# tuannv-github/srsRAN_Project

Hardware: AMD Instinct MI355X
Metric: PDSCH+PUSCH codeblocks/s @ 100 MHz 273-PRB 4x4 MIMO (PDSCH 4 layers, PUSCH 4 layers x 4 rx) (higher is better)
Workload: dtype int8+fp32; 1 GPU; BASELINE metric (PDSCH+PUSCH codeblocks/s @ 100 MHz 273-PRB 4x4 MIMO): full PDSCH+PUSCH slot pipeline, 100 MHz numerology-1 273 PRB, 256QAM R=948/1024; parallelism=single GPU

## Files before the change

### srsran_project_amd/csrc/ldpc_api.cpp

```cpp
#include "srsran_amd/ldpc.h"

#include <hip/hip_runtime.h>

#include "api_common.h"
#include "ldpc_codec_internal.h"
#include "ldpc_common.h"
#include <cstdarg>
#include <cstdio>
#include <cstring>
#include <mutex>
#include <string>
#include <algorithm>
#include <vector>

namespace srs_amd {


hipError_t launch_ldpc_decode(const decode_args& args, const lifted_graph& g, int arith, int grid, hipStream_t stream);
size_t     ldpc_decode_lds_bytes(const lifted_graph& g);

namespace {

constexpr int      MAX_CRC_BITS_LEN = 22 * MAX_LIFTING_SIZE;
constexpr uint32_t DEFAULT_SLOTS    = 1u << 20;
// ... 180 lines not shown
{
  return srs_amd::ldpc_decode_batch_ex(d, cfg, crc_poly, d_llrs, llr_stride, d_llr_lens, llr_len, d_output,
                                       out_stride, d_nof_iters, d_soft_out, nof_cbs, stream, nullptr, 0);
}

}

int srs_amd::ldpc_decode_batch_ex(srs_amd_ldpc_decoder*              d,
                                  const srs_amd_ldpc_decoder_config* cfg,
                                  int                                crc_poly,
                                  const int8_t*                      d_llrs,
                                  uint32_t                           llr_stride,
                                  const uint32_t*                    d_llr_lens,
                                  uint32_t                           llr_len,
                                  uint8_t*                           d_output,
                                  uint32_t                           out_stride,
                                  int32_t*                           d_nof_iters,
                                  int8_t*                            d_soft_out,
                                  uint32_t                           nof_cbs,
                                  void*                              stream,
                                  const uint8_t*                     d_skip_flags,
                                  uint32_t                           skip_stride,
                                  const int32_t*                     d_fillers,
                                  const ldpc_cw_rows*                cw)
{
  if (d == nullptr) {
    return fail(SRS_AMD_EINVAL, "null decoder");
  }
  int rc = validate(cfg, crc_poly);
  if (rc != SRS_AMD_OK) {
    return rc;
  }
  const uint32_t Z       = cfg->lifting_size;
  const uint32_t K       = (cfg->base_graph == 1 ? 22 : 10) * Z;
  const uint32_t N_short = (cfg->base_graph == 1 ? 66 : 50) * Z;
  if (nof_cbs == 0) {
    return SRS_AMD_OK;
  }
  if ((d_llrs == nullptr && cw == nullptr) || d_output == nullptr || d_nof_iters == nullptr ||
      (cw != nullptr && (cw->llrs == nullptr || cw->offsets == nullptr || cw->lengths == nullptr))) {
    return fail(SRS_AMD_EINVAL, "null device buffer");
  }
  if (cw != nullptr && (d_llr_lens != nullptr || d_soft_out != nullptr || d_skip_flags != nullptr || cw->qm == 0 ||
                        !ldpc_hr_takes(static_cast<int>(cfg->base_graph), static_cast<int>(cfg->lifting_size), llr_len))) {
    return fail(SRS_AMD_EINVAL, "codeword-fed rows need the high-rate decoder's configuration");
  }
  if (out_stride < (K + 7) / 8) {
// ... 27 lines not shown
  a.edges = d->edges + ((cfg->base_graph - 1) * NOF_LIFTING_SIZES + lifting_size_position(static_cast<int>(Z))) *
                             static_cast<size_t>(MAX_EDGES);
  a.llr_stride      = llr_stride;
  a.aligned4        = ((reinterpret_cast<uintptr_t>(d_llrs) | llr_stride) & 3u) == 0 ? 1 : 0;
  a.llr_len         = llr_len;
  a.out_stride      = out_stride;
  a.nof_cbs         = nof_cbs;
  a.nof_filler_bits = static_cast<int32_t>(cfg->nof_filler_bits);
  a.max_iterations  = static_cast<int32_t>(cfg->max_iterations);
  a.force_decoding  = d->force_decoding;
  a.skip_flags      = d_skip_flags;
  a.skip_stride     = skip_stride;
  a.fillers         = d_fillers;
  if (cw != nullptr) {
    a.llrs        = cw->llrs;
    a.aligned4    = 1;
    a.cw_llrs     = cw->llrs;
    a.cw_offsets  = cw->offsets;
    a.cw_lengths  = cw->lengths;
    a.cw_qm       = cw->qm;
    a.cw_nof_info = cw->nof_info;
    a.cw_filler   = cw->filler;
  }
  const int grid    = static_cast<int>(nof_cbs < d->max_slots ? nof_cbs : d->max_slots);
  e = launch_ldpc_decode(a, g, d->arith, grid, static_cast<hipStream_t>(stream));
  if (e != hipSuccess) {
    return hip_fail(e, "ldpc_decode_kernel launch");
  }
  return SRS_AMD_OK;
}

void srs_amd::ldpc_mixed_row(void* row, uint32_t bg, uint32_t Z, int crc_poly)
{
  ldpc_row_desc r{};
  r.Z        = Z;
  r.edge_off = static_cast<uint32_t>(lifted_edges_offset(static_cast<int>(bg), static_cast<int>(Z)));
  r.crc_off  = crc_poly == SRS_AMD_NO_CRC ? NO_CRC_ROW : static_cast<uint32_t>(crc_poly) * MAX_CRC_BITS_LEN;
  r.zmagic   = ldpc_z_magic(Z);
  std::memcpy(row, &r, sizeof(r));
}

int srs_amd::ldpc_decode_mixed(srs_amd_ldpc_decoder* d,
                               uint32_t              bg,
                               uint32_t              max_z,
                               uint32_t              max_iterations,
                               const int8_t*         d_llrs,
// ... 114 lines not shown
```

### srsran_project_amd/csrc/ldpc_codec_internal.h

```cpp
#pragma once

#include "srsran_amd/ldpc.h"
#include "srsran_amd/ldpc_encoder.h"
#include "srsran_amd/ldpc_rate_matching.h"

namespace srs_amd {

int rate_dematch_batch_ex(srs_amd_ldpc_rate_dematcher*      dm,
                          const srs_amd_codeblock_metadata* cfg,
                          int                               new_data,
                          const int8_t*                     d_input,
                          const uint32_t*                   d_in_offsets,
                          const uint32_t*                   d_rm_lengths,
                          int8_t*                           d_soft,
                          uint32_t                          soft_stride,
                          uint32_t                          nof_cbs,
                          void*                             stream,
                          bool                              fresh,
                          uint32_t                          write_end = 0);

int ldpc_encode_batch_ex(srs_amd_ldpc_encoder*              enc,
                         const srs_amd_ldpc_encoder_config* cfg,
                         const uint8_t*                     d_messages,
                         uint32_t                           msg_stride,
// ... 6 lines not shown
struct ldpc_cw_rows {
  const int8_t*   llrs;
  const uint32_t* offsets;
  const uint32_t* lengths;
  uint32_t        qm, nof_info, filler;
};

int ldpc_decode_batch_ex(srs_amd_ldpc_decoder*              d,
                         const srs_amd_ldpc_decoder_config* cfg,
                         int                                crc_poly,
                         const int8_t*                      d_llrs,
                         uint32_t                           llr_stride,
                         const uint32_t*                    d_llr_lens,
                         uint32_t                           llr_len,
                         uint8_t*                           d_output,
                         uint32_t                           out_stride,
                         int32_t*                           d_nof_iters,
                         int8_t*                            d_soft_out,
                         uint32_t                           nof_cbs,
                         void*                              stream,
                         const uint8_t*                     d_skip_flags,
                         uint32_t                           skip_stride,
                         const int32_t*                     d_fillers = nullptr,
                         const ldpc_cw_rows*                cw        = nullptr);

int ldpc_decode_mixed(srs_amd_ldpc_decoder* d,
                      uint32_t              bg,
                      uint32_t              max_z,
                      uint32_t              max_iterations,
                      const int8_t*         d_llrs,
                      uint32_t              llr_stride,
                      const uint32_t*       d_llr_lens,
                      uint8_t*              d_output,
                      uint32_t              out_stride,
                      int32_t*              d_nof_iters,
                      uint32_t              nof_cbs,
                      void*                 stream,
                      const int32_t*        d_fillers,
                      const void*           d_rows);

void ldpc_mixed_row(void* row, uint32_t bg, uint32_t Z, int crc_poly);

int ldpc_encode_mixed(srs_amd_ldpc_encoder* enc,
                      uint32_t              bg,
                      uint32_t              max_z,
                      uint32_t              max_rows_eff,
                      const uint8_t*        d_messages,
// ... 38 lines not shown
```

### srsran_project_amd/csrc/ldpc_common.h

```cpp
#pragma once

#include <cstddef>
#include <cstdint>
#include <vector>

namespace srs_amd {

constexpr int LLR_MAX      = 120;
constexpr int LLR_INFINITY = 127;
constexpr int SOFT_CLAMP = 64;

constexpr int MAX_LIFTING_SIZE = 384;
constexpr int MAX_BG_M         = 46;
constexpr int MAX_BG_N_FULL    = 68;
constexpr int MAX_EDGES        = 316;
constexpr int BG1_MAX_DEGREE   = 19;
constexpr int BG2_MAX_DEGREE   = 10;

enum arith_flavour : int {
  ARITH_SIMD = 0,
  ARITH_GENERIC = 1,
};

struct lifted_graph {
// ... 14 lines not shown
  uint8_t*        out;
  int32_t*        nof_iters;
  int8_t*         soft_out;
  const uint32_t* crc_table;
  const uint32_t* edges;
  uint32_t        llr_stride;
  uint32_t        llr_len;
  uint32_t        out_stride;
  uint32_t        nof_cbs;
  int32_t         nof_filler_bits;
  int32_t         max_iterations;
  int32_t         force_decoding;
  int32_t         aligned4;
  const uint8_t*  skip_flags;
  uint32_t        skip_stride;
  const int32_t*  fillers;
  const struct ldpc_row_desc* rows;
  const int8_t*   cw_llrs;
  const uint32_t* cw_offsets;
  const uint32_t* cw_lengths;
  uint32_t        cw_qm;
  uint32_t        cw_nof_info;
  uint32_t        cw_filler;
};

struct ldpc_row_desc {
  uint32_t Z;
  uint32_t edge_off;
  uint32_t crc_off;
  uint32_t zmagic;
};

uint32_t ldpc_z_magic(uint32_t Z);

bool ldpc_hr_takes(int bg, int Z, uint32_t llr_len);

int ldpc_pk_waves(int bg, int Z);
constexpr uint32_t NO_CRC_ROW = 0xffffffffu;
constexpr int32_t LDPC_ITERS_SKIPPED = -2;

int lifting_size_position(int Z);
constexpr int NOF_LIFTING_SIZES = 51;

bool build_lifted_graph(lifted_graph& g, int bg, int Z);

std::vector<uint32_t> all_lifted_edges();

// ... 13 lines not shown
```

### srsran_project_amd/csrc/ldpc_decoder.hip

```cpp
#include "kernel_probe.h"
#include "srsran_amd/profiling.h"
#include <hip/hip_runtime.h>

#include "ldpc_common.h"
#include <cstdlib>
#include <type_traits>
#include <utility>

namespace srs_amd {

#define SRS_BG_TABLE_QUAL constexpr
namespace tables {
#include "bg_tables.inc"
}
#undef SRS_BG_TABLE_QUAL

using const_u32_ptr = const __attribute__((address_space(4))) uint32_t*;

constexpr int LDS_RED_OFFSET  = 16;
constexpr int LDS_SOFT_OFFSET = 80;
using lds_i8                  = __attribute__((address_space(3))) int8_t;
using lds_i32                 = __attribute__((address_space(3))) int32_t;
using lds_u32                 = __attribute__((address_space(3))) uint32_t;

// ... 594 lines not shown

__device__ __forceinline__ pk16 pk_splat(int v)
{
  return pk16{static_cast<short>(v), static_cast<short>(v)};
}
__device__ __forceinline__ pk16 pk_min(pk16 a, pk16 b)
{
  return __builtin_elementwise_min(a, b);
}
__device__ __forceinline__ pk16 pk_max(pk16 a, pk16 b)
{
  return __builtin_elementwise_max(a, b);
}
__device__ __forceinline__ pk16 pk_clamp(pk16 x, int lim)
{
  return pk_min(pk_max(x, pk_splat(-lim)), pk_splat(lim));
}

template <int MAXL>
__host__ __device__ constexpr int hr_lds_bytes()
{
  return LDS_SOFT_OFFSET + (22 + MAXL) * HR_Z;
}

template <int EI, int H, int KOFF = 0>
__device__ __forceinline__ uint32_t hr_addr(uint32_t t)
{
  constexpr uint32_t s    = (const_edge<1, HR_Z, EI>::shift + H) % HR_Z;
  constexpr uint32_t base = LDS_SOFT_OFFSET + const_edge<1, HR_Z, EI>::var * HR_Z;
  if constexpr (s <= HR_HALF) {
    return t + (base + KOFF + s);
  } else {
    return __builtin_elementwise_min(t + (KOFF + s), t + (KOFF + s - HR_Z)) + base;
  }
}

template <int N, typename F, int... I>
__device__ __forceinline__ void static_for_impl(F&& f, std::integer_sequence<int, I...>)
{
  (f(std::integral_constant<int, I>{}), ...);
}
template <int N, typename F>
__device__ __forceinline__ void static_for(F&& f)
{
  static_for_impl<N>(f, std::make_integer_sequence<int, N>{});
}
// ... 564 lines not shown
  uint32_t l;
  asm volatile("v_mbcnt_lo_u32_b32 %0, -1, 0\n\tv_mbcnt_hi_u32_b32 %0, -1, %0" : "=v"(l));
  return wave_base + l;
}

template <int ARITH, int MAXL, int NP>
__global__ void __launch_bounds__(HR_HALF / NP, (hr_waves_per_simd<NP, MAXL>())) ldpc_decode_hr_kernel(decode_args a)
{
  constexpr bool FULL   = MAXL == bg_traits<1>::M;
  constexpr bool CMP    = FULL || (HR_CMP && NP == 1);
  static_assert(!FULL || NP == 1, "full-length codeblocks: one row pair per lane");
  constexpr int Z       = HR_Z;
  constexpr int K       = 22 * Z;
  constexpr int NODES   = 22 + MAXL;
  constexpr int NE      = row_start<1>(MAXL) * NP;
  constexpr int MAX_LLR = (NODES - 2) * Z;
  constexpr int NT      = HR_HALF / NP;
  lds_i32*      red     = (lds_i32*)(uintptr_t)LDS_RED_OFFSET;
  lds_i8*       lds     = (lds_i8*)(uintptr_t)0;
  lds_i8*       soft    = lds + LDS_SOFT_OFFSET;
  lds_i32*      soft4   = reinterpret_cast<lds_i32*>(soft);

  const uint32_t wave_base = __builtin_amdgcn_readfirstlane(threadIdx.x) & ~63u;
  for (uint32_t cb = blockIdx.x; cb < a.nof_cbs; cb += gridDim.x) {
    uint32_t t = hr_thread(wave_base);
    if (a.skip_flags && *reinterpret_cast<const int32_t*>(a.skip_flags + static_cast<size_t>(cb) * a.skip_stride)) {
      if (t == 0) {
        a.nof_iters[cb] = LDPC_ITERS_SKIPPED;
      }
      continue;
    }
    asm volatile("" : "+v"(t));
    const int8_t* in     = a.llrs + static_cast<size_t>(cb) * a.llr_stride;
    const int     n_llrs = static_cast<int>(a.llr_len);
    uint8_t*      out    = a.out + static_cast<size_t>(cb) * a.out_stride;

    if constexpr (NT > 64) {
      if (t == 0) {
        red[0] = -1;
        red[1] = 0;
        red[2] = 0;
      }
      __syncthreads();
    }
    int input_size;
    if (a.cw_llrs != nullptr) {
// ... 264 lines not shown
        if (crc != 0) {
          __hip_atomic_fetch_xor(&acc[0], crc, __ATOMIC_RELAXED, __HIP_MEMORY_SCOPE_WORKGROUP);
        }
        if (zero != 0) {
          __hip_atomic_fetch_or(&acc[1], 1u, __ATOMIC_RELAXED, __HIP_MEMORY_SCOPE_WORKGROUP);
        }
        __syncthreads();
        const uint32_t c_all = __builtin_amdgcn_readfirstlane(acc[0]);
        const uint32_t z_all = __builtin_amdgcn_readfirstlane(acc[1]);
        if (tq == 0) {
          lds_u32* nxt = reinterpret_cast<lds_u32*>(&red[1 + 2 * ((it + 1) & 1)]);
          nxt[0]       = 0;
          nxt[1]       = 0;
        }
        if (z_all == 0 && c_all == 0) {
          result = it + 1;
          break;
        }
      }
    }

    const uint32_t te = hr_thread(wave_base);
    static_assert(K % 128 == 0, "whole 16-byte hard-decision tasks");
    for (int task = te; task < K / 128; task += NT) {
      uint32_t o[4];
#pragma unroll
      for (int c = 0; c < 4; ++c) {
        o[c] = 0;
#pragma unroll
        for (int h = 0; h < 8; ++h) {
          const uint32_t w = static_cast<uint32_t>(soft4[32 * task + 8 * c + h]);
          const uint32_t d    = ((w | 0x80808080u) - 0x01010101u) ^ (~w & 0x80808080u);
          const uint32_t nib  = (((d & 0x80808080u) >> 7) * 0x08040201u) >> 24;
          const int      byte = h >> 1;
          o[c] |= (nib & 0xfu) << (8 * byte + ((h & 1) ? 0 : 4));
        }
      }
      uint8_t* ob = out + 16 * task;
      if (((reinterpret_cast<uintptr_t>(ob)) & 15u) == 0) {
        *reinterpret_cast<uint4*>(ob) = uint4{o[0], o[1], o[2], o[3]};
      } else {
#pragma unroll
        for (int b = 0; b < 16; ++b) {
          ob[b] = static_cast<uint8_t>(o[b >> 2] >> (8 * (b & 3)));
        }
      }
    }
    if (a.soft_out) {
      int32_t* so = reinterpret_cast<int32_t*>(a.soft_out + static_cast<size_t>(cb) * (68 * Z));
      for (int i = te; i < 68 * Z / 4; i += NT) {
        so[i] = i < NODES * Z / 4 ? static_cast<int32_t>(soft_export4(static_cast<uint32_t>(soft4[i]))) : 0;
      }
    }
    if (te == 0) {
      a.nof_iters[cb] = result;
    }
    if constexpr (NT > 64) {
      __syncthreads();
    } else {
      asm volatile("" ::: "memory");
    }
  }
}


template <int BG>
constexpr int pk_words(int l)
{
  return bg_traits<BG>::deg(l) > 13 ? 3 : 2;
}
template <int BG>
constexpr int pk_off(int l)
{
  int s = 0;
  for (int i = 0; i < l; ++i) {
    s += pk_words<BG>(i);
  }
  return s;
}
static_assert(pk_off<1>(46) == FR_STATE_WORDS && pk_off<2>(42) == 84, "compressed message state");

// ... 454 lines not shown
  const size_t lds = lds_total_bytes<BG>(g.Z);
  if (g.Z == 384) {
    hipLaunchKernelGGL((ldpc_decode_kernel<BG, ARITH, 384>), dim3(grid), dim3(max_threads<384>()), lds, stream, args, g);
  } else {
    hipLaunchKernelGGL((ldpc_decode_kernel<BG, ARITH, 0>), dim3(grid), dim3(threads), lds, stream, args, g);
  }
}

bool ldpc_hr_takes(int bg, int Z, uint32_t llr_len)
{
  static const bool enabled = [] {
    const char* e = std::getenv("SRSRAN_AMD_LDPC_HR");
    return e == nullptr || e[0] != '0';
  }();
  return enabled && bg == 1 && Z == HR_Z && llr_len <= static_cast<uint32_t>((20 + HR_MAXL) * HR_Z) &&
         (llr_len & 3u) == 0;
}

hipError_t launch_ldpc_decode(const decode_args& args, const lifted_graph& g, int arith, int grid, hipStream_t stream)
{
  if (args.cw_llrs != nullptr && !(ldpc_decode_hr_eligible(args, g) && ldpc_hr_takes(g.bg, g.Z, args.llr_len))) {
    return hipErrorInvalidValue;
  }
  if (ldpc_decode_hr_eligible(args, g)) {
    constexpr size_t lds = hr_lds_bytes<HR_MAXL>();
    constexpr int    NT  = HR_HALF / HR_NP;
    if (arith == ARITH_GENERIC) {
      SRS_PROBED_LAUNCH(SRS_AMD_PROBE_LDPC_HR, (ldpc_decode_hr_kernel<ARITH_GENERIC, HR_MAXL, HR_NP>), dim3(grid),
                        dim3(NT), lds, stream, args);
    } else {
      SRS_PROBED_LAUNCH(SRS_AMD_PROBE_LDPC_HR, (ldpc_decode_hr_kernel<ARITH_SIMD, HR_MAXL, HR_NP>), dim3(grid),
                        dim3(NT), lds, stream, args);
    }
    return hipGetLastError();
  }
  if (ldpc_decode_full_eligible(args, g)) {
    constexpr int    MAXL = bg_traits<1>::M;
    constexpr size_t lds  = hr_lds_bytes<MAXL>();
    if (arith == ARITH_GENERIC) {
      SRS_PROBED_LAUNCH(SRS_AMD_PROBE_LDPC_FULL, (ldpc_decode_hr_kernel<ARITH_GENERIC, MAXL, 1>), dim3(grid),
                        dim3(HR_HALF), lds, stream, args);
    } else {
      SRS_PROBED_LAUNCH(SRS_AMD_PROBE_LDPC_FULL, (ldpc_decode_hr_kernel<ARITH_SIMD, MAXL, 1>), dim3(grid),
                        dim3(HR_HALF), lds, stream, args);
    }
    return hipGetLastError();
  }
  const int pkw = ldpc_pk_waves(g.bg, g.Z);
  if (pkw > 0 && !(g.bg == 1 && g.Z == HR_Z) && (reinterpret_cast<uintptr_t>(args.soft_out) & 3u) == 0) {
// ... 28 lines not shown
```

### srsran_project_amd/csrc/ldpc_graph.cpp

```cpp
#include "ldpc_common.h"

#include <algorithm>

namespace srs_amd {

#include "bg_tables.inc"

int lifting_index(int Z)
{
  static const int odd_to_ils[16] = {-1, 0, -1, 1, -1, 2, -1, 3, -1, 4, -1, 5, -1, 6, -1, 7};
  if (Z < 2 || Z > MAX_LIFTING_SIZE) {
    return -1;
  }
  int a = Z;
  while ((a & 1) == 0) {
    a >>= 1;
  }
  return (a > 15) ? -1 : odd_to_ils[a];
}

int lifting_size_position(int Z)
{
  static const int sizes[NOF_LIFTING_SIZES] = {2,   3,   4,   5,   6,   7,   8,   9,   10,  11,  12,  13,  14,
                                               15,  16,  18,  20,  22,  24,  26,  28,  30,  32,  36,  40,  44,
// ... 68 lines not shown
{
  uint32_t polynom = 0;
  int      order   = 0;
  crc_params(poly, polynom, order);
  std::vector<uint32_t> t(nbits);
  const uint64_t        highbit = 1ull << order;
  uint64_t              r       = 1;
  for (int i = 0; i < order; ++i) {
    r <<= 1;
    if (r & highbit) {
      r ^= polynom;
    }
  }
  for (int k = 0; k < nbits; ++k) {
    t[k] = static_cast<uint32_t>(r & (highbit - 1));
    r <<= 1;
    if (r & highbit) {
      r ^= polynom;
    }
  }
  return t;
}

bool crc_params(int poly, uint32_t& polynom, int& order)
{
  switch (poly) {
    case 0: order = 24; polynom = 0x1864cfb; return true;
    case 1: order = 24; polynom = 0x1800063; return true;
    case 2: order = 24; polynom = 0x1b2b117; return true;
    case 3: order = 16; polynom = 0x11021; return true;
    case 4: order = 11; polynom = 0xe21; return true;
    case 5: order = 6; polynom = 0x61; return true;
    default: return false;
  }
}

}
```

### srsran_project_amd/csrc/pusch_api.cpp

```cpp
#include "srsran_amd/crc.h"
#include "srsran_amd/ldpc.h"
#include "srsran_amd/ldpc_rate_matching.h"
#include "srsran_amd/sch.h"

#include <hip/hip_runtime.h>

#include "api_common.h"
#include "crc_internal.h"
#include "device_buffer.h"
#include "ldpc_codec_internal.h"
#include "ldpc_common.h"
#include "rate_matching_common.h"
#include "pusch_processor_args.h"
#include "sch_args.h"
#include <cstring>
#include <algorithm>
#include <map>
#include <mutex>
#include <tuple>
#include <vector>

using namespace srs_amd;

struct srs_amd_pusch_decoder {
  int                          device = 0;
  int                          arith  = 0;
  hipStream_t                  stream = nullptr;
  srs_amd_crc_calculator*      crc[3] = {nullptr, nullptr, nullptr};
  srs_amd_ldpc_rate_dematcher* dm     = nullptr;
  srs_amd_ldpc_decoder*        dec[2] = {nullptr, nullptr};
  device_buffer                soft, msgs, iters, checks, arrays, results, host_io, tb_acc, slot_desc;
  device_buffer                harq_prev;
  geometry_cache               rm_geo;
  stream_order                 order;
  stream_fan                   fan;
  std::mutex                   mtx;
  pinned_stage hstage;
  ~srs_amd_pusch_decoder()
  {
    (void)hipSetDevice(device);
    if (stream) {
      (void)hipStreamSynchronize(stream);
      (void)hipStreamDestroy(stream);
    }
    for (auto* c : crc) {
      srs_amd_crc_calculator_destroy(c);
    }
    srs_amd_ldpc_rate_dematcher_destroy(dm);
    srs_amd_ldpc_decoder_destroy(dec[0]);
    srs_amd_ldpc_decoder_destroy(dec[1]);
  }
};

namespace {
// ... 68 lines not shown
  const uint32_t        rows       = nof_tbs * C;
  const soft_row_layout lay        = layout_of(p);
  const uint32_t        msg_stride = static_cast<uint32_t>(align_up((p->segment_length + 7) / 8, 64));
  const bool            internal   = d_soft == nullptr;
  hipError_t            he         = hipSetDevice(d->device);
  if (internal && he == hipSuccess) {
    he     = d->soft.ensure(static_cast<size_t>(rows) * lay.row_bytes);
    d_soft = d->soft.as<int8_t>();
  }
  if (he == hipSuccess) {
    he = d->msgs.ensure(static_cast<size_t>(rows) * msg_stride);
  }
  if (he == hipSuccess) {
    he = d->iters.ensure(sizeof(int32_t) * rows);
  }
  if (he == hipSuccess) {
    he = d->checks.ensure(sizeof(uint32_t) * rows);
  }
  if (he == hipSuccess) {
    he = d->arrays.ensure(sizeof(uint32_t) * 2 * rows);
  }
  if (he == hipSuccess) {
    he = d->tb_acc.ensure_zeroed(sizeof(uint32_t) * nof_tbs);
  }
  if (he != hipSuccess) {
    return hip_fail(he, "PUSCH decoder scratch");
  }
  call_scope scope(d->order, nullptr, stream);
  he = d->order.begin(stream);
  if (he == hipSuccess) {
    const uint32_t key[6] = {nof_tbs, C, p->nof_short_segments, p->rm_length_short, p->rm_length_long, llr_stride};
    if (d->rm_geo.stale(d->arrays.ptr, key, 6)) {
      he = launch_rm_arrays(d->arrays.as<uint32_t>(), nof_tbs, C, p->nof_short_segments, p->rm_length_short,
                            p->rm_length_long, llr_stride, stream);
      if (he != hipSuccess) {
        d->rm_geo.invalidate();
      }
    }
  }
  if (he != hipSuccess) {
    return hip_fail(he, "PUSCH decoder rate-matching arrays");
  }
  srs_amd_codeblock_metadata md{p->base_graph, p->lifting_size, p->rv, p->modulation_order, p->Nref,
                                p->nof_filler_bits};
  const uint32_t prefix = llr_prefix(p, lay, cfg->new_data != 0, internal);
  ldpc_cw_rows cw{};
// ... 7 lines not shown
           g.k0 == 0 && e_max <= g.L && e_max + g.F <= prefix;
    cw = ldpc_cw_rows{d_llrs, d->arrays.as<uint32_t>() + rows, d->arrays.as<uint32_t>(), p->modulation_order,
                      g.nof_info, g.F};
  }
  int rc = SRS_AMD_OK;
  if (!fuse) {
    rc = rate_dematch_batch_ex(d->dm, &md, cfg->new_data ? 1 : 0, d_llrs, d->arrays.as<uint32_t>() + rows,
                               d->arrays.as<uint32_t>(), d_soft, lay.row_bytes, rows, stream, internal,
                               internal ? prefix : 0);
  }
  if (rc != SRS_AMD_OK) {
    return rc;
  }
  const int crc_index = crc_index_of(p);
  const int crc_poly  = crc_poly_of(p);
  srs_amd_ldpc_decoder_config dc{};
  dc.base_graph      = p->base_graph;
  dc.lifting_size    = p->lifting_size;
  dc.nof_filler_bits = p->nof_filler_bits;
  dc.nof_crc_bits    = C > 1 ? p->nof_crc_bits : p->nof_tb_crc_bits;
  dc.max_iterations  = cfg->nof_ldpc_iterations;
  srs_amd_ldpc_decoder* dec = d->dec[cfg->force_decoding ? 1 : 0];
  const bool skip = !cfg->new_data && !internal;
  rc = ldpc_decode_batch_ex(dec, &dc, cfg->use_early_stop ? crc_poly : SRS_AMD_NO_CRC, d_soft, lay.row_bytes, nullptr,
                            prefix, d->msgs.as<uint8_t>(), msg_stride,
                            d->iters.as<int32_t>(), nullptr, rows, stream,
                            skip ? reinterpret_cast<const uint8_t*>(d_soft) + lay.flag_offset : nullptr, lay.row_bytes,
                            nullptr, fuse ? &cw : nullptr);
  if (rc != SRS_AMD_OK) {
    return rc;
  }
  if (!cfg->use_early_stop) {
    rc = srs_amd_crc_calculate_batch(d->crc[crc_index], d->checks.as<uint32_t>(), d->msgs.as<uint8_t>(), msg_stride,
                                     p->segment_length - p->nof_filler_bits, rows, stream);
    if (rc != SRS_AMD_OK) {
      return rc;
    }
  }
  assemble_args a{};
  a.msgs           = d->msgs.as<uint8_t>();
  a.iters          = d->iters.as<int32_t>();
  a.crc_checks     = cfg->use_early_stop ? nullptr : d->checks.as<uint32_t>();
  a.soft           = internal ? nullptr : reinterpret_cast<uint8_t*>(d_soft);
  a.tbs            = d_tbs;
  a.results        = d_results;
  a.cb_iterations  = d_cb_iterations;
  a.crc24a_table   = crc_device_table(d->crc[1]);
  a.acc            = d->tb_acc.as<uint32_t>();
  a.lay            = lay;
  a.msg_stride     = msg_stride;
  a.tb_stride      = tb_stride;
  a.nof_segments   = C;
  a.cb_info_bits   = p->cb_info_bits;
  a.tbs_bits       = p->tbs;
  a.max_iterations = cfg->nof_ldpc_iterations;
  a.new_data       = cfg->new_data ? 1 : 0;
  he               = launch_assemble(a, nof_tbs, stream);
  if (he == hipSuccess) {
    he = scope.close();
  }
  return he == hipSuccess ? SRS_AMD_OK : hip_fail(he, "assemble_kernel launch");
}

int decode_slot_locked(srs_amd_pusch_decoder*              d,
                       const srs_amd_pusch_decoder_config* cfg,
                       const srs_amd_pusch_ue*             ues,
                       uint32_t                            U,
                       const int8_t*                       d_llrs,
                       uint8_t*                            d_tbs,
                       srs_amd_pusch_decoder_result*       d_results,
                       const uint32_t*                     cb_offsets,
                       int32_t*                            d_cb_iterations,
                       hipStream_t                         stream,
                       const slot_harq*                    harq,
                       const slot_ue_patch*                patches,
                       uint32_t                            nof_patches)
{
  auto harq_of = [&](uint32_t u) -> const slot_harq* {
    return harq != nullptr && harq[u].soft != nullptr ? &harq[u] : nullptr;
// ... 352 lines not shown
  if (rc != SRS_AMD_OK) {
    return rc;
  }
  auto* d   = new srs_amd_pusch_decoder();
  d->device = device;
  d->arith  = arith;
  rc        = srs_amd_crc_calculator_create(&d->crc[0], 3, 8448, device);
  if (rc == SRS_AMD_OK) {
    rc = srs_amd_crc_calculator_create(&d->crc[1], 0, 1277992, device);
  }
  if (rc == SRS_AMD_OK) {
    rc = srs_amd_crc_calculator_create(&d->crc[2], 1, 8448, device);
  }
  if (rc == SRS_AMD_OK) {
    rc = srs_amd_ldpc_rate_dematcher_create(&d->dm, device);
  }
  if (rc == SRS_AMD_OK) {
    rc = srs_amd_ldpc_decoder_create(&d->dec[0], arith, 0, device);
  }
  if (rc == SRS_AMD_OK) {
    rc = srs_amd_ldpc_decoder_create(&d->dec[1], arith, 1, device);
  }
  if (rc == SRS_AMD_OK) {
    hipError_t he = hipStreamCreateWithFlags(&d->stream, hipStreamNonBlocking);
    if (he != hipSuccess) {
      rc = hip_fail(he, "PUSCH decoder stream");
    }
  }
  if (rc != SRS_AMD_OK) {
    delete d;
    return rc;
  }
  *out = d;
  return SRS_AMD_OK;
}

void srs_amd_pusch_decoder_destroy(srs_amd_pusch_decoder* dec)
{
  delete dec;
}

int srs_amd_pusch_soft_buffer_layout(const srs_amd_sch_plan* plan, uint32_t* row_bytes, uint32_t* nof_llrs,
                                     uint32_t* msg_offset, uint32_t* flag_offset)
{
  const int rc = check_plan(plan);
  if (rc != SRS_AMD_OK) {
// ... 186 lines not shown
```

### srsran_project_amd/csrc/sch.hip

```cpp
#include <hip/hip_runtime.h>

#include <cstdlib>

#include "crc_device.h"
#include "sch_args.h"

namespace srs_amd {
namespace {

constexpr int SEG_THREADS = 256;
constexpr int ASM_THREADS = 256;
constexpr uint32_t CRC24A_POLY = 0x1864cfb;
constexpr uint32_t SCH_MAX_SEGMENTS = 512;
constexpr uint32_t ASM_TB_PER       = 32;
constexpr uint32_t ASM_TB_CHUNK     = ASM_THREADS * ASM_TB_PER;

__device__ __forceinline__ uint32_t bit_at(const uint8_t* b, uint32_t p)
{
  return (b[p >> 3] >> (7 - (p & 7))) & 1u;
}

__device__ __forceinline__ uint8_t segment_byte(const uint8_t* tb, uint32_t tb_off, uint32_t n_data, bool last,
                                                uint32_t crc, uint32_t tb_crc_bits, uint32_t j)
{
// ... 259 lines not shown
  return {a.tbs + static_cast<size_t>(t) * a.tb_stride, t * a.nof_segments, a.nof_segments, a.cb_info_bits,
          a.tbs_bits};
}

__device__ __forceinline__ void assemble_tb(const assemble_args& a, uint32_t t, bool zero_acc)
{
  __shared__ uint32_t s_ok, s_sum, s_min, s_max, s_tb_ok;
  __shared__ uint8_t  s_fresh[SCH_MAX_SEGMENTS];
  __shared__ uint8_t  s_cb_ok[SCH_MAX_SEGMENTS];
  __shared__ uint16_t s_stat[SCH_MAX_SEGMENTS];
  const tb_view       v = view_of(a, t);
  if (zero_acc && threadIdx.x == 0 && a.acc != nullptr) {
    a.acc[t] = 0;
  }
  const uint32_t      C = v.C;
  if (threadIdx.x == 0) {
    s_ok    = 0;
    s_sum   = 0;
    s_min   = 0xffffffffu;
    s_max   = 0;
    s_tb_ok = 0;
  }
  __syncthreads();
  for (uint32_t r = threadIdx.x; r < C; r += ASM_THREADS) {
    const uint32_t cb   = v.row0 + r;
    const uint8_t* srow = a.soft ? a.soft + static_cast<size_t>(cb) * a.lay.row_bytes : nullptr;
    const int32_t  flag = srow && !a.new_data ? *reinterpret_cast<const int32_t*>(srow + a.lay.flag_offset) : 0;
    const bool     prev = flag != 0;
    const int32_t  it   = a.iters[cb];
    const bool     dec  = !prev && (a.crc_checks ? (a.crc_checks[cb] == 0) : (it >= 0));
    const uint32_t stat = prev  ? static_cast<uint32_t>(flag)
                          : dec ? (a.crc_checks ? a.max_iterations : static_cast<uint32_t>(it))
                                : a.max_iterations;
    const bool     ok   = prev || dec;
    s_fresh[r]          = prev ? 0 : 1;
    s_cb_ok[r]          = ok ? 1 : 0;
    if (a.cb_iterations) {
      a.cb_iterations[a.tds != nullptr ? a.tds[t].pad + r : cb] = ok ? static_cast<int32_t>(stat) : -1;
    }
    if (!prev && a.soft) {
      s_stat[r] = stat;
    }
    atomicAdd(&s_ok, ok ? 1u : 0u);
    atomicAdd(&s_sum, stat);
    atomicMin(&s_min, stat);
    atomicMax(&s_max, stat);
  }
  __syncthreads();
  const uint8_t* src = a.msgs + static_cast<size_t>(v.row0) * a.msg_stride;
  if (a.soft) {
    for (uint32_t r = threadIdx.x; r < C; r += ASM_THREADS) {
      if (s_fresh[r]) {
        *reinterpret_cast<int32_t*>(a.soft + static_cast<size_t>(v.row0 + r) * a.lay.row_bytes + a.lay.flag_offset) =
            s_cb_ok[r] ? static_cast<int32_t>(s_stat[r]) : 0;
      }
    }
    __syncthreads();
    src = a.soft + static_cast<size_t>(v.row0) * a.lay.row_bytes + a.lay.msg_offset;
  }
  uint8_t*       tb     = v.tb;
  const uint32_t nbytes = v.tbs_bits / 8;
  const bool     all_ok = s_ok == C;
  if (C == 1) {
    if (all_ok) {
      for (uint32_t j = threadIdx.x; j < nbytes; j += ASM_THREADS) {
        tb[j] = src[j];
      }
    }
    if (threadIdx.x == 0) {
      s_tb_ok = all_ok ? 1 : 0;
    }
  }
  __syncthreads();
  if (threadIdx.x == 0) {
    srs_amd_pusch_decoder_result res{};
    res.tb_crc_ok             = static_cast<int32_t>(s_tb_ok);
    res.nof_codeblocks_total  = C;
    res.ldpc_iterations_sum   = s_sum;
    res.ldpc_iterations_min   = s_min;
    res.ldpc_iterations_max   = s_max;
    res.nof_codeblocks_crc_ok = s_ok;
    a.results[t]              = res;
  }
}

__global__ __launch_bounds__(ASM_THREADS) void assemble_kernel(assemble_args a)
{
  assemble_tb(a, blockIdx.x, true);
}

__device__ __forceinline__ const uint8_t* asm_source(const assemble_args& a, const tb_view& v, uint32_t& stride)
{
  if (a.soft) {
// ... 72 lines not shown
  const uint32_t to = min(v.tbs_bits, (c0 + ASM_TB_CHUNK) * 8);
  const uint32_t x  = crc_block_xor<ASM_THREADS>(
      crc_chunk_contrib(lds_fetch{s_chunk, c0}, b0, b1, v.tbs_bits, 24, CRC24A_POLY, a.crc24a_table, T, to),
      partial);
  if (threadIdx.x == 0 && x != 0) {
    atomicXor(a.acc + t, crc_move(x, v.tbs_bits - to, 24, a.crc24a_table));
  }
}

__global__ __launch_bounds__(ASM_THREADS) void asm_tb_kernel(assemble_args a)
{
  asm_tb_chunk(a, blockIdx.y, blockIdx.x, true);
}

__global__ __launch_bounds__(ASM_THREADS) void asm_merged_kernel(assemble_args a)
{
  if (blockIdx.x == gridDim.x - 1) {
    assemble_tb(a, blockIdx.y, false);
  } else {
    asm_tb_chunk(a, blockIdx.y, blockIdx.x, false);
  }
}

__global__ __launch_bounds__(64) void asm_final_kernel(assemble_args a, uint32_t nof_tbs)
{
  const uint32_t t = blockIdx.x * 64 + threadIdx.x;
  if (t >= nof_tbs) {
    return;
  }
  const tb_view  v = view_of(a, t);
  const uint32_t C = v.C;
  const uint32_t acc = a.acc != nullptr ? a.acc[t] : 0u;
  if (a.acc != nullptr) {
    a.acc[t] = 0;
  }
  if (C == 1 || a.results[t].nof_codeblocks_crc_ok != C) {
    return;
  }
  uint32_t       stride;
  const uint8_t* src = asm_source(a, v, stride);
  const uint32_t off = v.tbs_bits - (C - 1) * v.cbi;
  const uint8_t* m   = src + static_cast<size_t>(C - 1) * stride;
  uint32_t       chk = 0;
  for (uint32_t k = 0; k < 24; ++k) {
    chk = (chk << 1) | bit_at(m, off + k);
  }
// ... 196 lines not shown
  }
  dim3 grid((a.msg_bytes + SEG_THREADS - 1) / SEG_THREADS, a.nof_rows);
  hipLaunchKernelGGL(segment_kernel, grid, dim3(SEG_THREADS), 0, stream, a);
  return hipGetLastError();
}

hipError_t launch_tx_slot_segment(const tx_slot_args& a, hipStream_t stream)
{
  if (a.nof_tbs == 0) {
    return hipSuccess;
  }
  hipError_t e = hipMemsetAsync(a.acc, 0, sizeof(uint32_t) * a.nof_tbs, stream);
  if (e != hipSuccess) {
    return e;
  }
  hipLaunchKernelGGL(tx_tb_crc_kernel, dim3((a.max_tb_bytes + ASM_TB_CHUNK - 1) / ASM_TB_CHUNK, a.nof_tbs),
                     dim3(ASM_THREADS), 0, stream, a);
  hipLaunchKernelGGL(tx_segment_kernel, dim3((a.max_msg_bytes + SEG_THREADS - 1) / SEG_THREADS, a.nof_rows),
                     dim3(SEG_THREADS), 0, stream, a);
  hipLaunchKernelGGL(tx_cb_crc_kernel, dim3(a.nof_rows), dim3(64), 0, stream, a);
  return hipGetLastError();
}

hipError_t launch_assemble(const assemble_args& a, uint32_t nof_tbs, hipStream_t stream)
{
  if (nof_tbs == 0) {
    return hipSuccess;
  }
  if (a.soft) {
    const uint32_t nw  = (a.lay.flag_offset - a.lay.msg_offset + 3) / 4;
    const uint32_t ncb = nof_tbs * a.nof_segments;
    hipLaunchKernelGGL(asm_copy_kernel, dim3((ncb * nw + ASM_THREADS - 1) / ASM_THREADS), dim3(ASM_THREADS), 0,
                       stream, a, ncb, nw);
  }
  const uint32_t nbytes = (a.tds != nullptr ? a.max_tb_bits : a.tbs_bits) / 8;
  const char*    mv     = std::getenv("SRSRAN_AMD_ASM_MERGED");
  if (a.soft == nullptr && !(a.tds == nullptr && a.nof_segments == 1) && !(mv != nullptr && mv[0] == '0')) {
    hipLaunchKernelGGL(asm_merged_kernel, dim3((nbytes + ASM_TB_CHUNK - 1) / ASM_TB_CHUNK + 1, nof_tbs),
                       dim3(ASM_THREADS), 0, stream, a);
    hipError_t e = hipGetLastError();
    if (e != hipSuccess) {
      return e;
    }
    hipLaunchKernelGGL(asm_final_kernel, dim3((nof_tbs + 63) / 64), dim3(64), 0, stream, a, nof_tbs);
    return hipGetLastError();
  }
  hipLaunchKernelGGL(assemble_kernel, dim3(nof_tbs), dim3(ASM_THREADS), 0, stream, a);
  hipError_t e = hipGetLastError();
  if (e != hipSuccess || (a.tds == nullptr && a.nof_segments == 1)) {
    return e;
  }
  hipLaunchKernelGGL(asm_tb_kernel, dim3((nbytes + ASM_TB_CHUNK - 1) / ASM_TB_CHUNK, nof_tbs), dim3(ASM_THREADS), 0,
                     stream, a);
  e = hipGetLastError();
  if (e != hipSuccess) {
    return e;
  }
  hipLaunchKernelGGL(asm_final_kernel, dim3((nof_tbs + 63) / 64), dim3(64), 0, stream, a, nof_tbs);
// ... 5 lines not shown
```

### srsran_project_amd/csrc/sch_args.h

```cpp
#pragma once

#include <hip/hip_runtime.h>

#include <cstdint>

#include "srsran_amd/sch.h"

namespace srs_amd {

struct rm_geometry;
struct enc_row_desc;

struct segment_args {
  const uint8_t*  tbs;
  const uint32_t* tb_crcs;
  uint8_t*        msgs;
  uint32_t        tb_stride;
  uint32_t        msg_stride;
  uint32_t        msg_bytes;
  uint32_t        nof_segments;
  uint32_t        cb_info_bits;
  uint32_t        last_data_bits;
  uint32_t        tb_crc_bits;
  uint32_t        nof_rows;
// ... 63 lines not shown
};
hipError_t launch_pdsch_fused(const pdsch_fused_args& a, hipStream_t stream);

struct assemble_args {
  const uint8_t*                msgs;
  const int32_t*                iters;
  const uint32_t*               crc_checks;
  uint8_t*                      soft;
  uint8_t*                      tbs;
  srs_amd_pusch_decoder_result* results;
  int32_t*                      cb_iterations;
  const uint32_t*               crc24a_table;
  uint32_t*                     acc;
  soft_row_layout               lay;
  uint32_t                      msg_stride;
  uint32_t                      tb_stride;
  uint32_t                      nof_segments;
  uint32_t                      cb_info_bits;
  uint32_t                      tbs_bits;
  uint32_t                      max_iterations;
  int32_t                       new_data;
  const tb_desc*                tds;
  uint32_t                      max_tb_bits;
};

struct harq_row_desc {
  uint8_t* soft_row;
  uint32_t row;
  uint32_t soft_bytes;
  uint32_t msg_offset;
  uint32_t msg_bytes;
  uint32_t flag_offset;
  uint32_t new_data;
  uint32_t lazy;
  uint32_t tb_row0;
  uint32_t tb_C;
};
struct harq_tb_desc {
  uint8_t* soft;
  uint32_t result;
  uint32_t C;
  uint32_t row_bytes;
  uint32_t flag_offset;
  uint32_t lazy;
  uint32_t row0;
  uint32_t soft_bytes;
// ... 11 lines not shown
  int32_t*                      prev;
  srs_amd_pusch_decoder_result* results;
};
hipError_t launch_harq_gather(const harq_args& a, uint32_t max_soft_bytes, hipStream_t stream);
hipError_t launch_harq_scatter(const harq_args& a, uint32_t max_soft_bytes, hipStream_t stream);
hipError_t launch_harq_final(const harq_args& a, hipStream_t stream);

struct slot_row_patch {
  uint32_t*       row_E;
  uint32_t*       row_in;
  const int32_t*  sel;
  const uint32_t* cand_E;
  const uint32_t* cand_off;
  uint32_t        llr_offset;
  uint32_t        C;
};
hipError_t launch_slot_row_patch(const slot_row_patch* items, uint32_t n, hipStream_t stream);

hipError_t launch_segment(const segment_args& a, hipStream_t stream);
bool       segment_attaches_crc(const segment_args& a);
hipError_t launch_rm_arrays(uint32_t* arrays, uint32_t nof_tbs, uint32_t C, uint32_t nof_short, uint32_t e_short,
                            uint32_t e_long, uint32_t tb_units, hipStream_t stream);
hipError_t launch_assemble(const assemble_args& a, uint32_t nof_tbs, hipStream_t stream);

}
```

Before: 24.97 million codeblocks/s.

## Compute per-codeblock TB CRC partials in LDPC decoder and fuse assemble copy

During hard-decision output, the LDPC decoder now computes each codeblock's partial CRC24A contribution using slice-by-4 and precomputed x^n multiplication tables, then reduces it across the wave and block. The assemble stage combines these partials with crc_move to check the transport-block CRC, so it no longer re-runs CRC over the whole TB. It also uses a new fused kernel that copies message bytes in parallel word chunks. This adds table lookups in the decoder epilogue and a gated, more complex assemble path that only applies under strict segment-size conditions.

```diff
diff --git a/srsran_project_amd/csrc/ldpc_api.cpp b/srsran_project_amd/csrc/ldpc_api.cpp
--- a/srsran_project_amd/csrc/ldpc_api.cpp
+++ b/srsran_project_amd/csrc/ldpc_api.cpp
@@ -226,7 +226,10 @@
                                   const uint8_t*                     d_skip_flags,
                                   uint32_t                           skip_stride,
                                   const int32_t*                     d_fillers,
-                                  const ldpc_cw_rows*                cw)
+                                  const ldpc_cw_rows*                cw,
+                                  uint32_t*                          d_tb_partial,
+                                  const uint32_t*                    d_tb_crc_table,
+                                  uint32_t                           tb_partial_bits)
 {
   if (d == nullptr) {
     return fail(SRS_AMD_EINVAL, "null decoder");
@@ -300,6 +303,9 @@
     a.cw_nof_info = cw->nof_info;
     a.cw_filler   = cw->filler;
   }
+  a.tb_partial      = d_tb_partial;
+  a.tb_crc_table    = d_tb_crc_table;
+  a.tb_partial_bits = tb_partial_bits;
   const int grid    = static_cast<int>(nof_cbs < d->max_slots ? nof_cbs : d->max_slots);
   e = launch_ldpc_decode(a, g, d->arith, grid, static_cast<hipStream_t>(stream));
   if (e != hipSuccess) {
diff --git a/srsran_project_amd/csrc/ldpc_codec_internal.h b/srsran_project_amd/csrc/ldpc_codec_internal.h
--- a/srsran_project_amd/csrc/ldpc_codec_internal.h
+++ b/srsran_project_amd/csrc/ldpc_codec_internal.h
@@ -52,7 +52,10 @@
                          const uint8_t*                     d_skip_flags,
                          uint32_t                           skip_stride,
                          const int32_t*                     d_fillers = nullptr,
-                         const ldpc_cw_rows*                cw        = nullptr);
+                         const ldpc_cw_rows*                cw        = nullptr,
+                         uint32_t*                          d_tb_partial    = nullptr,
+                         const uint32_t*                    d_tb_crc_table  = nullptr,
+                         uint32_t                           tb_partial_bits = 0);
 
 int ldpc_decode_mixed(srs_amd_ldpc_decoder* d,
                       uint32_t              bg,
diff --git a/srsran_project_amd/csrc/ldpc_common.h b/srsran_project_amd/csrc/ldpc_common.h
--- a/srsran_project_amd/csrc/ldpc_common.h
+++ b/srsran_project_amd/csrc/ldpc_common.h
@@ -60,7 +60,21 @@
   uint32_t        cw_qm;
   uint32_t        cw_nof_info;
   uint32_t        cw_filler;
+  uint32_t*       tb_partial;
+  const uint32_t* tb_crc_table;
+  uint32_t        tb_partial_bits;
 };
+
+constexpr uint32_t TBP_SLICE     = 0;
+constexpr uint32_t TBP_MUL_WORDS = 3 * 256;
+constexpr uint32_t TBP_NOF_LO    = 8;
+constexpr uint32_t TBP_NOF_HI    = 9;
+constexpr uint32_t TBP_NOF_TAIL  = 17;
+constexpr uint32_t TBP_LO        = TBP_SLICE + 4 * 256;
+constexpr uint32_t TBP_HI        = TBP_LO + TBP_NOF_LO * TBP_MUL_WORDS;
+constexpr uint32_t TBP_TAIL      = TBP_HI + TBP_NOF_HI * TBP_MUL_WORDS;
+constexpr uint32_t TBP_WORDS     = TBP_TAIL + TBP_NOF_TAIL * TBP_MUL_WORDS;
+std::vector<uint32_t> tb_partial_tables(int poly);
 
 struct ldpc_row_desc {
   uint32_t Z;
diff --git a/srsran_project_amd/csrc/ldpc_decoder.hip b/srsran_project_amd/csrc/ldpc_decoder.hip
--- a/srsran_project_amd/csrc/ldpc_decoder.hip
+++ b/srsran_project_amd/csrc/ldpc_decoder.hip
@@ -640,6 +640,7 @@
 {
   return LDS_SOFT_OFFSET + (22 + MAXL) * HR_Z;
 }
+constexpr int HR_TB_LDS_BYTES = 16;
 
 template <int EI, int H, int KOFF = 0>
 __device__ __forceinline__ uint32_t hr_addr(uint32_t t)
@@ -1250,6 +1251,7 @@
   lds_i32*      soft4   = reinterpret_cast<lds_i32*>(soft);
 
   const uint32_t wave_base = __builtin_amdgcn_readfirstlane(threadIdx.x) & ~63u;
+  lds_u32* tb_w = (lds_u32*)(uintptr_t)hr_lds_bytes<MAXL>();
   for (uint32_t cb = blockIdx.x; cb < a.nof_cbs; cb += gridDim.x) {
     uint32_t t = hr_thread(wave_base);
     if (a.skip_flags && *reinterpret_cast<const int32_t*>(a.skip_flags + static_cast<size_t>(cb) * a.skip_stride)) {
@@ -1560,6 +1562,7 @@
 
     const uint32_t te = hr_thread(wave_base);
     static_assert(K % 128 == 0, "whole 16-byte hard-decision tasks");
+    uint32_t tb_x = 0;
     for (int task = te; task < K / 128; task += NT) {
       uint32_t o[4];
 #pragma unroll
@@ -1583,6 +1586,60 @@
           ob[b] = static_cast<uint8_t>(o[b >> 2] >> (8 * (b & 3)));
         }
       }
+      if constexpr (!FULL) {
+        if (a.tb_partial != nullptr) {
+          const uint32_t* T  = a.tb_crc_table;
+          const int       nb = static_cast<int>(a.tb_partial_bits >> 3);
+          const int       b0 = 16 * task;
+          if (b0 < nb) {
+            uint32_t r = 0;
+#pragma unroll
+            for (int c = 0; c < 4; ++c) {
+              const uint32_t w = __builtin_bswap32(o[c]);
+              if (b0 + 4 * c + 4 <= nb) {
+                r = T[TBP_SLICE + 768 + (r >> 16)] ^ T[TBP_SLICE + 512 + ((r >> 8) & 0xffu)] ^
+                    T[TBP_SLICE + 256 + (r & 0xffu)] ^ T[TBP_SLICE + (w >> 24)] ^ (w & 0xffffffu);
+              } else {
+#pragma unroll
+                for (int k = 0; k < 3; ++k) {
+                  if (b0 + 4 * c + k < nb) {
+                    r = T[TBP_SLICE + (r >> 16)] ^ ((r << 8) & 0xffffffu) ^ ((w >> (24 - 8 * k)) & 0xffu);
+                  }
+                }
+              }
+            }
+            const int  last = (nb - 1) >> 4;
+            const bool mv   = task < last;
+            const int  m    = mv ? last - 1 - task : 0;
+            const int  n    = mv ? nb - 16 * last : 0;
+            const uint32_t* M[3] = {T + TBP_LO + TBP_MUL_WORDS * static_cast<uint32_t>(m & 7),
+                                    T + TBP_HI + TBP_MUL_WORDS * static_cast<uint32_t>(m >> 3),
+                                    T + TBP_TAIL + TBP_MUL_WORDS * static_cast<uint32_t>(n)};
+#pragma unroll
+            for (int s = 0; s < 3; ++s) {
+              r = M[s][r & 0xffu] ^ M[s][256 + ((r >> 8) & 0xffu)] ^ M[s][512 + (r >> 16)];
+            }
+            tb_x ^= r;
+          }
+        }
+      }
+    }
+    if constexpr (!FULL) {
+      if (a.tb_partial != nullptr) {
+        uint32_t x = tb_x;
+#pragma unroll
+        for (uint32_t o = 32; o >= 1; o >>= 1) {
+          x ^= static_cast<uint32_t>(
+              __builtin_amdgcn_ds_bpermute(static_cast<int>(((te ^ o) & 63u) << 2), static_cast<int>(x)));
+        }
+        if ((te & 63u) == 0) {
+          if constexpr (NT == 64) {
+            a.tb_partial[cb] = x;
+          } else {
+            tb_w[wave_base >> 6] = x;
+          }
+        }
+      }
     }
     if (a.soft_out) {
       int32_t* so = reinterpret_cast<int32_t*>(a.soft_out + static_cast<size_t>(cb) * (68 * Z));
@@ -1595,6 +1652,16 @@
     }
     if constexpr (NT > 64) {
       __syncthreads();
+      if constexpr (!FULL) {
+        if (a.tb_partial != nullptr && hr_thread(wave_base) == 0) {
+          uint32_t x = 0;
+#pragma unroll
+          for (int w = 0; w < NT / 64; ++w) {
+            x ^= tb_w[w];
+          }
+          a.tb_partial[cb] = x;
+        }
+      }
     } else {
       asm volatile("" ::: "memory");
     }
@@ -2095,9 +2162,14 @@
   if (args.cw_llrs != nullptr && !(ldpc_decode_hr_eligible(args, g) && ldpc_hr_takes(g.bg, g.Z, args.llr_len))) {
     return hipErrorInvalidValue;
   }
+  if (args.tb_partial != nullptr &&
+      !(ldpc_decode_hr_eligible(args, g) && args.tb_crc_table != nullptr && args.tb_partial_bits % 8 == 0 &&
+        args.tb_partial_bits <= 22u * HR_Z)) {
+    return hipErrorInvalidValue;
+  }
   if (ldpc_decode_hr_eligible(args, g)) {
-    constexpr size_t lds = hr_lds_bytes<HR_MAXL>();
-    constexpr int    NT  = HR_HALF / HR_NP;
+    const size_t  lds = hr_lds_bytes<HR_MAXL>() + (args.tb_partial != nullptr ? HR_TB_LDS_BYTES : 0);
+    constexpr int NT  = HR_HALF / HR_NP;
     if (arith == ARITH_GENERIC) {
       SRS_PROBED_LAUNCH(SRS_AMD_PROBE_LDPC_HR, (ldpc_decode_hr_kernel<ARITH_GENERIC, HR_MAXL, HR_NP>), dim3(grid),
                         dim3(NT), lds, stream, args);
diff --git a/srsran_project_amd/csrc/ldpc_graph.cpp b/srsran_project_amd/csrc/ldpc_graph.cpp
--- a/srsran_project_amd/csrc/ldpc_graph.cpp
+++ b/srsran_project_amd/csrc/ldpc_graph.cpp
@@ -114,6 +114,55 @@
   return t;
 }
 
+std::vector<uint32_t> tb_partial_tables(int poly)
+{
+  uint32_t polynom = 0;
+  int      order   = 0;
+  crc_params(poly, polynom, order);
+  auto times_x = [&](uint32_t r, int n) {
+    for (int i = 0; i < n; ++i) {
+      r <<= 1;
+      if (r & 0x1000000u) {
+        r ^= polynom;
+      }
+    }
+    return r;
+  };
+  auto mulmod = [&](uint32_t a, uint32_t c) {
+    uint32_t r = 0;
+    for (int i = 0; i < 24; ++i) {
+      if ((a >> i) & 1u) {
+        r ^= c;
+      }
+      c = times_x(c, 1);
+    }
+    return r;
+  };
+  std::vector<uint32_t> t(TBP_WORDS);
+  for (uint32_t k = 0; k < 4; ++k) {
+    for (uint32_t b = 0; b < 256; ++b) {
+      t[TBP_SLICE + 256 * k + b] = times_x(b, 24 + 8 * static_cast<int>(k));
+    }
+  }
+  auto fill = [&](uint32_t at, uint32_t c) {
+    for (uint32_t k = 0; k < 3; ++k) {
+      for (uint32_t b = 0; b < 256; ++b) {
+        t[at + 256 * k + b] = mulmod(b << (8 * k), c);
+      }
+    }
+  };
+  for (uint32_t i = 0; i < TBP_NOF_LO; ++i) {
+    fill(TBP_LO + TBP_MUL_WORDS * i, times_x(1, 128 * static_cast<int>(i)));
+  }
+  for (uint32_t i = 0; i < TBP_NOF_HI; ++i) {
+    fill(TBP_HI + TBP_MUL_WORDS * i, times_x(1, 128 * static_cast<int>(TBP_NOF_LO * i)));
+  }
+  for (uint32_t i = 0; i < TBP_NOF_TAIL; ++i) {
+    fill(TBP_TAIL + TBP_MUL_WORDS * i, times_x(1, 8 * static_cast<int>(i)));
+  }
+  return t;
+}
+
 bool crc_params(int poly, uint32_t& polynom, int& order)
 {
   switch (poly) {
diff --git a/srsran_project_amd/csrc/pusch_api.cpp b/srsran_project_amd/csrc/pusch_api.cpp
--- a/srsran_project_amd/csrc/pusch_api.cpp
+++ b/srsran_project_amd/csrc/pusch_api.cpp
@@ -30,6 +30,8 @@
   srs_amd_ldpc_rate_dematcher* dm     = nullptr;
   srs_amd_ldpc_decoder*        dec[2] = {nullptr, nullptr};
   device_buffer                soft, msgs, iters, checks, arrays, results, host_io, tb_acc, slot_desc;
+  device_buffer                cb_parts;
+  device_buffer                tb_tabs;
   device_buffer                harq_prev;
   geometry_cache               rm_geo;
   stream_order                 order;
@@ -144,6 +146,9 @@
   }
   if (he == hipSuccess) {
     he = d->tb_acc.ensure_zeroed(sizeof(uint32_t) * nof_tbs);
+  }
+  if (he == hipSuccess) {
+    he = d->cb_parts.ensure(sizeof(uint32_t) * rows);
   }
   if (he != hipSuccess) {
     return hip_fail(he, "PUSCH decoder scratch");
@@ -197,11 +202,15 @@
   dc.max_iterations  = cfg->nof_ldpc_iterations;
   srs_amd_ldpc_decoder* dec = d->dec[cfg->force_decoding ? 1 : 0];
   const bool skip = !cfg->new_data && !internal;
+  const bool partials = internal && cfg->use_early_stop &&
+                        ldpc_hr_takes(static_cast<int>(p->base_graph), static_cast<int>(p->lifting_size), prefix) &&
+                        assemble_takes_partials(C, p->cb_info_bits, p->tbs);
   rc = ldpc_decode_batch_ex(dec, &dc, cfg->use_early_stop ? crc_poly : SRS_AMD_NO_CRC, d_soft, lay.row_bytes, nullptr,
                             prefix, d->msgs.as<uint8_t>(), msg_stride,
                             d->iters.as<int32_t>(), nullptr, rows, stream,
                             skip ? reinterpret_cast<const uint8_t*>(d_soft) + lay.flag_offset : nullptr, lay.row_bytes,
-                            nullptr, fuse ? &cw : nullptr);
+                            nullptr, fuse ? &cw : nullptr, partials ? d->cb_parts.as<uint32_t>() : nullptr,
+                            partials ? d->tb_tabs.as<uint32_t>() : nullptr, partials ? p->cb_info_bits : 0u);
   if (rc != SRS_AMD_OK) {
     return rc;
   }
@@ -230,6 +239,7 @@
   a.tbs_bits       = p->tbs;
   a.max_iterations = cfg->nof_ldpc_iterations;
   a.new_data       = cfg->new_data ? 1 : 0;
+  a.cb_partials    = partials ? d->cb_parts.as<uint32_t>() : nullptr;
   he               = launch_assemble(a, nof_tbs, stream);
   if (he == hipSuccess) {
     he = scope.close();
@@ -628,6 +638,16 @@
     rc = srs_amd_ldpc_decoder_create(&d->dec[1], arith, 1, device);
   }
   if (rc == SRS_AMD_OK) {
+    const std::vector<uint32_t> t  = tb_partial_tables(0);
+    hipError_t                  he = d->tb_tabs.ensure(sizeof(uint32_t) * t.size());
+    if (he == hipSuccess) {
+      he = hipMemcpy(d->tb_tabs.ptr, t.data(), sizeof(uint32_t) * t.size(), hipMemcpyHostToDevice);
+    }
+    if (he != hipSuccess) {
+      rc = hip_fail(he, "PUSCH decoder CRC tables");
+    }
+  }
+  if (rc == SRS_AMD_OK) {
     hipError_t he = hipStreamCreateWithFlags(&d->stream, hipStreamNonBlocking);
     if (he != hipSuccess) {
       rc = hip_fail(he, "PUSCH decoder stream");
diff --git a/srsran_project_amd/csrc/sch.hip b/srsran_project_amd/csrc/sch.hip
--- a/srsran_project_amd/csrc/sch.hip
+++ b/srsran_project_amd/csrc/sch.hip
@@ -305,6 +305,7 @@
     s_tb_ok = 0;
   }
   __syncthreads();
+  uint32_t tb_x = 0;
   for (uint32_t r = threadIdx.x; r < C; r += ASM_THREADS) {
     const uint32_t cb   = v.row0 + r;
     const uint8_t* srow = a.soft ? a.soft + static_cast<size_t>(cb) * a.lay.row_bytes : nullptr;
@@ -316,6 +317,9 @@
                           : dec ? (a.crc_checks ? a.max_iterations : static_cast<uint32_t>(it))
                                 : a.max_iterations;
     const bool     ok   = prev || dec;
+    if (C > 1 && a.cb_partials != nullptr) {
+      tb_x ^= crc_move(a.cb_partials[cb], (C - 1 - r) * v.cbi, 24, a.crc24a_table);
+    }
     s_fresh[r]          = prev ? 0 : 1;
     s_cb_ok[r]          = ok ? 1 : 0;
     if (a.cb_iterations) {
@@ -352,6 +356,12 @@
     }
     if (threadIdx.x == 0) {
       s_tb_ok = all_ok ? 1 : 0;
+    }
+  } else if (a.cb_partials != nullptr) {
+    __shared__ uint32_t s_part[ASM_THREADS / 64];
+    const uint32_t      x = crc_block_xor<ASM_THREADS>(tb_x, s_part);
+    if (threadIdx.x == 0) {
+      s_tb_ok = (all_ok && x == 0) ? 1 : 0;
     }
   }
   __syncthreads();
@@ -470,6 +480,76 @@
   }
 }
 
+constexpr uint32_t ASM_CP_WORDS = ASM_TB_CHUNK / 4;
+constexpr uint32_t ASM_CP_U     = ASM_CP_WORDS / ASM_THREADS;
+
+__device__ __forceinline__ void asm_copy_runs(uint8_t* tb, const uint8_t* src, uint32_t stride, uint32_t cbB,
+                                              uint32_t nbytes, uint32_t chunk, const int32_t* iters, uint32_t C)
+{
+  const int32_t it0 = threadIdx.x < C ? iters[threadIdx.x] : 0;
+  const uint32_t mis = static_cast<uint32_t>(reinterpret_cast<uintptr_t>(tb) & 3u);
+  uint32_t*      tbw = reinterpret_cast<uint32_t*>(tb - mis);
+  const uint32_t nw  = (nbytes + mis + 3) / 4;
+  const uint32_t w0  = chunk * ASM_CP_WORDS + threadIdx.x;
+  uint32_t       lo[ASM_CP_U], hi[ASM_CP_U], sh[ASM_CP_U];
+  bool           whole[ASM_CP_U];
+#pragma unroll
+  for (uint32_t u = 0; u < ASM_CP_U; ++u) {
+    const uint32_t w = w0 + u * ASM_THREADS;
+    whole[u]         = false;
+    lo[u] = hi[u] = sh[u] = 0;
+    if (w < nw && 4 * w >= mis && 4 * w - mis + 4 <= nbytes) {
+      const uint32_t j = 4 * w - mis;
+      const uint32_t r = j / cbB;
+      const uint32_t o = j - r * cbB;
+      if (o + 4 <= cbB) {
+        const uint8_t* s = src + static_cast<size_t>(r) * stride + o;
+        const uint32_t k = static_cast<uint32_t>(reinterpret_cast<uintptr_t>(s) & 3u);
+        const uint32_t* sw = reinterpret_cast<const uint32_t*>(s - k);
+        whole[u]          = true;
+        lo[u]             = sw[0];
+        hi[u]             = k != 0 ? sw[1] : 0u;
+        sh[u]             = 8 * k;
+      }
+    }
+  }
+  int bad = it0 < 0 ? 1 : 0;
+  for (uint32_t r = threadIdx.x + ASM_THREADS; r < C; r += ASM_THREADS) {
+    bad |= iters[r] < 0 ? 1 : 0;
+  }
+  if (__syncthreads_or(bad) != 0) {
+    return;
+  }
+#pragma unroll
+  for (uint32_t u = 0; u < ASM_CP_U; ++u) {
+    const uint32_t w = w0 + u * ASM_THREADS;
+    if (whole[u]) {
+      tbw[w] = static_cast<uint32_t>(((static_cast<uint64_t>(hi[u]) << 32) | lo[u]) >> sh[u]);
+    } else if (w < nw) {
+      for (uint32_t b = 0; b < 4; ++b) {
+        const uint32_t p = 4 * w + b;
+        if (p >= mis && p - mis < nbytes) {
+          const uint32_t j = p - mis;
+          const uint32_t r = j / cbB;
+          tb[j]            = src[static_cast<size_t>(r) * stride + (j - r * cbB)];
+        }
+      }
+    }
+  }
+}
+
+__global__ __launch_bounds__(ASM_THREADS) void asm_fused_kernel(assemble_args a)
+{
+  const uint32_t t = blockIdx.y;
+  if (blockIdx.x == gridDim.x - 1) {
+    assemble_tb(a, t, false);
+    return;
+  }
+  const tb_view v = view_of(a, t);
+  asm_copy_runs(v.tb, a.msgs + static_cast<size_t>(v.row0) * a.msg_stride, a.msg_stride, v.cbi / 8, v.tbs_bits / 8,
+                blockIdx.x, a.iters + v.row0, v.C);
+}
+
 __global__ __launch_bounds__(64) void asm_final_kernel(assemble_args a, uint32_t nof_tbs)
 {
   const uint32_t t = blockIdx.x * 64 + threadIdx.x;
@@ -712,6 +792,13 @@
   return hipGetLastError();
 }
 
+bool assemble_takes_partials(uint32_t nof_segments, uint32_t cb_info_bits, uint32_t tbs_bits)
+{
+  const char* e = std::getenv("SRSRAN_AMD_ASM_FUSED");
+  return !(e != nullptr && e[0] == '0') && nof_segments > 1 && cb_info_bits % 8 == 0 &&
+         static_cast<uint64_t>(nof_segments) * cb_info_bits == static_cast<uint64_t>(tbs_bits) + 24;
+}
+
 hipError_t launch_assemble(const assemble_args& a, uint32_t nof_tbs, hipStream_t stream)
 {
   if (nof_tbs == 0) {
@@ -724,6 +811,15 @@
                        stream, a, ncb, nw);
   }
   const uint32_t nbytes = (a.tds != nullptr ? a.max_tb_bits : a.tbs_bits) / 8;
+  if (a.cb_partials != nullptr) {
+    if (a.soft != nullptr || a.tds != nullptr || a.crc_checks != nullptr || a.nof_segments < 2 ||
+        a.cb_info_bits % 8 != 0 || a.nof_segments * a.cb_info_bits != a.tbs_bits + 24) {
+      return hipErrorInvalidValue;
+    }
+    const uint32_t chunks = ((nbytes + 3 + 3) / 4 + ASM_CP_WORDS - 1) / ASM_CP_WORDS;
+    hipLaunchKernelGGL(asm_fused_kernel, dim3(chunks + 1, nof_tbs), dim3(ASM_THREADS), 0, stream, a);
+    return hipGetLastError();
+  }
   const char*    mv     = std::getenv("SRSRAN_AMD_ASM_MERGED");
   if (a.soft == nullptr && !(a.tds == nullptr && a.nof_segments == 1) && !(mv != nullptr && mv[0] == '0')) {
     hipLaunchKernelGGL(asm_merged_kernel, dim3((nbytes + ASM_TB_CHUNK - 1) / ASM_TB_CHUNK + 1, nof_tbs),
diff --git a/srsran_project_amd/csrc/sch_args.h b/srsran_project_amd/csrc/sch_args.h
--- a/srsran_project_amd/csrc/sch_args.h
+++ b/srsran_project_amd/csrc/sch_args.h
@@ -109,6 +109,7 @@
   int32_t                       new_data;
   const tb_desc*                tds;
   uint32_t                      max_tb_bits;
+  const uint32_t*               cb_partials;
 };
 
 struct harq_row_desc {
@@ -166,5 +167,6 @@
 hipError_t launch_rm_arrays(uint32_t* arrays, uint32_t nof_tbs, uint32_t C, uint32_t nof_short, uint32_t e_short,
                             uint32_t e_long, uint32_t tb_units, hipStream_t stream);
 hipError_t launch_assemble(const assemble_args& a, uint32_t nof_tbs, hipStream_t stream);
+bool       assemble_takes_partials(uint32_t nof_segments, uint32_t cb_info_bits, uint32_t tbs_bits);
 
 }
```

Result: no change. 25.12 million codeblocks/s, median of 6 (+0.6%).
